# GPUEngineering/RapidNet

Measured on AMD Instinct MI355X. Metric: apg_iterations_per_sec, higher is better.
Workload: dtype f64; 1 GPU; barcelona493: nx=63 nu=114 nv=97 nd=88 N=24 K=493 nodes=10864; operator_storage=dense per-node blocks (reference storage model), parallelism=1 GPU

## Files before the change

rapidnet_amd/csrc/k_stream.hpp:

```cpp
#pragma once
#include "common.hpp"
#include "stream_bits.hpp"

namespace rn {

__device__ __forceinline__ bool stream_nz(double v) { return ((unsigned long long)__double_as_longlong(v) << 1) != 0ull; }
__device__ __forceinline__ bool stream_nz(float v) { return (__float_as_uint(v) << 1) != 0u; }
__host__ __device__ constexpr int stream_vmcnt(int n) { return (n & 15) | ((n >> 4) << 14) | 0x0F70; }
#define RN_LANDED(n) __builtin_amdgcn_s_waitcnt(stream_vmcnt(n));
#define RN_LOADG(buf, sv) _Pragma("unroll") for (int d = 0; d < RN_GROUP; d++) { RN_POP(sv, d) RN_LOAD1(buf, sv, d) }
#define RN_USEG(buf, sv) _Pragma("unroll") for (int d = 0; d < RN_GROUP; d++) RN_USE1(buf, sv, d)
#define RN_LOADH(buf, sv) _Pragma("unroll") for (int d = 0; d < RN_GROUP - 1; d++) if (d < nHead) { RN_POP(sv, d) RN_LOAD1(buf, sv, d) }
#define RN_USEH(buf, sv) _Pragma("unroll") for (int d = 0; d < RN_GROUP - 1; d++) if (d < nHead) RN_USE1(buf, sv, d)
#define RN_STREAM_GROUPS                                                                                               \
    RN_LOADH(bufB, sB)                                                                                                 \
    if (nGroups > 0) RN_LOADG(bufA, sA)                                                                                \
    RN_USEH(bufB, sB)                                                                                                  \
    if (nGroups > 0) {                                                                                                 \
        RN_LANDED(RN_GROUP_LOADS)                                                                                      \
        int g = 0;                                                                                                     \
        for (; g + 2 < nGroups; g += 2) {                                                                              \
            RN_LOADG(bufB, sB)                                                                                         \
            RN_USEG(bufA, sA)                                                                                          \
            RN_LOADG(bufA, sA)                                                                                         \
            RN_USEG(bufB, sB)                                                                                          \
        }                                                                                                              \
        if (g + 1 < nGroups) {                                                                                         \
            RN_LOADG(bufB, sB)                                                                                         \
            RN_USEG(bufA, sA)                                                                                          \
            RN_USEG(bufB, sB)                                                                                          \
        } else {                                                                                                       \
            RN_USEG(bufA, sA)                                                                                          \
        }                                                                                                              \
    }                                                                                                                  \
    RN_LANDED(0)
template <typename T, typename VT, int VPL, int NL, int D, int NR>
__device__ __forceinline__ void stream_walk(const VT *__restrict__ Ab, const T *sh_y, const T *sh_y2, const unsigned long long *sh_nz, int skip, int span0, int span1, int G, int ny,
                                            int spanSlots, const int (&off)[NL], const int (&cj)[NL], const T (&msk)[NL], T (&part)[NL][VPL],
                                            T (&part2)[NR == 2 ? NL : 1][VPL], int &liveSpans, int &liveCols, int &liveRagged) {
    const int lane = threadIdx.x & 63;
    const int rag = (ny % G != 0 && span1 * G > ny) ? ny / G : -1;
    VT bufA[D][NL], bufB[D][NL];
    int sA[D], sB[D];
    liveSpans = 0; liveCols = 0; liveRagged = 0;
    const char *const Abb = reinterpret_cast<const char *>(Ab);
    const unsigned spanBytes = (unsigned)spanSlots * 16u;
    unsigned offB[NL];
#pragma unroll
    for (int j = 0; j < NL; j++) offB[j] = (unsigned)off[j] * 16u;
#define RN_POP(sv, d) { sv[d] = __builtin_amdgcn_readfirstlane(cb + __builtin_ctzll(mf)); mf &= mf - 1ull; }
#define RN_GROUP D
#define RN_GROUP_LOADS (D * NL)
#define RN_LOAD1(buf, sv, d)                                                                                           \
    _Pragma("unroll") for (int j = 0; j < NL; j++)                                                                     \
        buf[d][j] = __builtin_nontemporal_load(reinterpret_cast<const VT *>(Abb + (size_t)sv[d] * spanBytes + offB[j]));
#define RN_USE1(buf, sv, d)                                                                                            \
    _Pragma("unroll") for (int j = 0; j < NL; j++) {                                                                   \
        const T yc = sh_y[sv[d] * G + cj[j]] * msk[j];                                                                 \
        _Pragma("unroll") for (int e = 0; e < VPL; e++) part[j][e] += (T)buf[d][j][e] * yc;                            \
        if (NR == 2) {       \
            const T yc2 = sh_y2[sv[d] * G + cj[j]] * msk[j];                                                           \
            _Pragma("unroll") for (int e = 0; e < VPL; e++) part2[j][e] += (T)buf[d][j][e] * yc2;                      \
        }                                                                                                              \
    }
    for (int cb = span0; cb < span1; cb += 64) {
        const int s = cb + lane;
        int cols = 0;
        if (s < span1) {
            const int c0 = s * G;
            if (skip) {
                cols = __popcll(stream_mask_bits(sh_nz, c0, G));
            } else {
                cols = ny - c0 < G ? ny - c0 : G;
            }
        }
        const unsigned long long m = __ballot(cols > 0);
        liveSpans += __popcll(m);
        if (threadIdx.x < 64) {
            int t = cols;
#pragma unroll
            for (int o = 32; o > 0; o >>= 1) t += __shfl_xor(t, o);
            liveCols += t;
        }
        const unsigned long long ragBit = (rag >= cb && rag < cb + 64) ? (m & (1ull << (rag - cb))) : 0ull;
        unsigned long long mf = m & ~ragBit;
        const int nLive = __popcll(mf), nGroups = nLive / D, nHead = nLive - nGroups * D;
        RN_STREAM_GROUPS
        if (ragBit) {
            liveRagged = 1;
            VT bufR[NL];
#pragma unroll
            for (int j = 0; j < NL; j++) {
                const bool ok = msk[j] != (T)0 && rag * G + cj[j] < ny;
                bufR[j] = __builtin_nontemporal_load(reinterpret_cast<const VT *>(Abb + (size_t)rag * spanBytes + (ok ? offB[j] : 0u)));
            }
#pragma unroll
            for (int j = 0; j < NL; j++) {
                const int c = rag * G + cj[j];
                const bool ok = msk[j] != (T)0 && c < ny;
                const T yc = ok ? sh_y[c] : (T)0;
#pragma unroll
                for (int e = 0; e < VPL; e++) part[j][e] += (T)bufR[j][e] * yc;
                if (NR == 2) {
                    const T yc2 = ok ? sh_y2[c] : (T)0;
#pragma unroll
                    for (int e = 0; e < VPL; e++) part2[j][e] += (T)bufR[j][e] * yc2;
                }
            }
        }
    }
#undef RN_GROUP
#undef RN_GROUP_LOADS
#undef RN_POP
#undef RN_LOAD1
#undef RN_USE1
}
template <typename T, typename VT, int VPL, int DU, int NR>
__device__ __forceinline__ void stream_walk_half(const VT *__restrict__ Ab, const T *sh_y, const T *sh_y2, const unsigned long long *sh_nz, int skip, int halfOn, int span0, int span1,
                                                 int G, int ny, int spanSlots, const int (&off)[2], const int (&cj)[2], const T (&msk)[2], T (&part)[2][VPL],
                                                 T (&part2)[NR == 2 ? 2 : 1][VPL], int &liveSpans, int &liveCols, int &liveRagged, int &liveUnits) {
    const int lane = threadIdx.x & 63, Gh = G >> 1;
    const int u0 = 2 * span0, u1 = 2 * span1;
    const int rag = (ny % G != 0 && span1 * G > ny) ? ny / G : -1;
    VT bufA[DU], bufB[DU];
    int sA[DU], sB[DU];
    liveSpans = 0; liveCols = 0; liveRagged = 0; liveUnits = 0;
    const char *const Abb = reinterpret_cast<const char *>(Ab);
    const unsigned spanBytes = (unsigned)spanSlots * 16u;
    const unsigned offB[2] = {(unsigned)off[0] * 16u, (unsigned)off[1] * 16u};
#define RN_GROUP DU
#define RN_GROUP_LOADS DU
#define RN_POP(sv, d) { sv[d] = __builtin_amdgcn_readfirstlane(ub + __builtin_ctzll(mf)); mf &= mf - 1ull; }
#define RN_LOAD1(buf, sv, d) buf[d] = __builtin_nontemporal_load(reinterpret_cast<const VT *>(Abb + (size_t)(sv[d] >> 1) * spanBytes + ((sv[d] & 1) ? offB[1] : offB[0])));
#define RN_USE1(buf, sv, d) {                                                                                          \
        const bool h1 = (sv[d] & 1) != 0;                                                                              \
        const int cy = (sv[d] >> 1) * G + (h1 ? cj[1] : cj[0]);                                                        \
        const T yv = sh_y[cy];                                                                                         \
        const T ya = h1 ? (T)0 : yv, yb = h1 ? yv : (T)0;                                                              \
        _Pragma("unroll") for (int e = 0; e < VPL; e++) { part[0][e] += (T)buf[d][e] * ya; part[1][e] += (T)buf[d][e] * yb; } \
        if (NR == 2) {                                                                                                 \
            const T yv2 = sh_y2[cy];                                                                                   \
            const T ya2 = h1 ? (T)0 : yv2, yb2 = h1 ? yv2 : (T)0;                                                      \
            _Pragma("unroll") for (int e = 0; e < VPL; e++) { part2[0][e] += (T)buf[d][e] * ya2; part2[NR == 2 ? 1 : 0][e] += (T)buf[d][e] * yb2; } \
        }                                                                                                              \
    }
    for (int ub = u0; ub < u1; ub += 64) {
        const int u = ub + lane;
        const int c0 = halfOn ? u * Gh : (u >> 1) * G, n = halfOn ? Gh : G;
        int cols = 0;
        if (u < u1 && c0 < ny) cols = skip ? __popcll(stream_mask_bits(sh_nz, c0, n)) : (ny - c0 < n ? ny - c0 : n);
        const unsigned long long m = __ballot(cols > 0);
        liveSpans += __popcll((m | (m >> 1)) & 0x5555555555555555ull);
        liveUnits += __popcll(m);
        if (threadIdx.x < 64) {
            int t = (halfOn || !(lane & 1)) ? cols : 0;
#pragma unroll
            for (int o = 32; o > 0; o >>= 1) t += __shfl_xor(t, o);
            liveCols += t;
        }
        const int ragSh = 2 * rag - ub;
        const unsigned long long ragBits = (ragSh >= 0 && ragSh < 64) ? (m & (3ull << ragSh)) : 0ull;
        unsigned long long mf = m & ~ragBits;
        const int nLive = __popcll(mf), nGroups = nLive / DU, nHead = nLive - nGroups * DU;
        RN_STREAM_GROUPS
        if (ragBits) {
            liveRagged = 1;
#pragma unroll
            for (int h = 0; h < 2; h++)
                if ((ragBits >> (ragSh + h)) & 1ull) {
                    if (halfOn) { const int left = ny - (2 * rag + h) * Gh; liveUnits += (1 << 16) + ((left < Gh ? left : Gh) << 20); }
                    const int c = rag * G + cj[h];
                    const bool ok = msk[h] != (T)0 && c < ny;
                    const VT bufR = __builtin_nontemporal_load(reinterpret_cast<const VT *>(Abb + (ok ? (size_t)rag * spanBytes + offB[h] : (size_t)0)));
                    const T yc = ok ? sh_y[c] : (T)0;
#pragma unroll
                    for (int e = 0; e < VPL; e++) part[h][e] += (T)bufR[e] * yc;
                    if (NR == 2) {
                        const T yc2 = ok ? sh_y2[c] : (T)0;
#pragma unroll
                        for (int e = 0; e < VPL; e++) part2[NR == 2 ? h : 0][e] += (T)bufR[e] * yc2;
                    }
                }
        }
    }
#undef RN_GROUP
#undef RN_GROUP_LOADS
#undef RN_POP
#undef RN_LOAD1
#undef RN_USE1
#undef RN_LOADG
#undef RN_USEG
#undef RN_LOADH
#undef RN_USEH
#undef RN_STREAM_GROUPS
#undef RN_LANDED
}
template <typename T, int NL>
__device__ __forceinline__ void stream_slots(int tid, int G, int SPC, int spanSlots, int (&off)[NL], int (&cj)[NL], T (&msk)[NL]) {
    const bool halves = NL == 2 && !(G & 1);
    const int stride = halves ? spanSlots >> 1 : STREAM_THREADS;
#pragma unroll
    for (int j = 0; j < NL; j++) {
        const int q = tid + stride * j;
        const bool ok = halves ? tid < stride : q < spanSlots;
        off[j] = ok ? q : (halves ? stride * (j + 1) - 1 : spanSlots - 1);
        cj[j] = off[j] / SPC;
        msk[j] = ok ? (T)1 : (T)0;
    }
}
template <typename T, typename VT, int VPL, int DU, int NR>
__device__ __forceinline__ void stream_walk_two(const VT *__restrict__ Ab, const T *sh_y, const T *sh_y2, const unsigned long long *sh_nz, int skip, int halfOn, int span0, int span1,
                                                int G, int ny, int spanSlots, const int (&off)[2], const int (&cj)[2], const T (&msk)[2],
                                                T (&part)[2][VPL], T (&part2)[NR == 2 ? 2 : 1][VPL], int &liveSpans, int &liveCols, int &liveRagged, int &liveUnits) {
    liveSpans = 0; liveCols = 0; liveRagged = 0; liveUnits = 0;
    const int firstIdle = (G & 1) ? STREAM_THREADS : spanSlots >> 1;
    if (__builtin_amdgcn_readfirstlane((int)threadIdx.x & ~63) < firstIdle)
        stream_walk_half<T, VT, VPL, DU, NR>(Ab, sh_y, sh_y2, sh_nz, skip, (G & 1) ? 0 : halfOn, span0, span1, G, ny, spanSlots, off, cj, msk, part, part2,
                                            liveSpans, liveCols, liveRagged, liveUnits);
}
template <typename T, int NR>
__device__ __forceinline__ void stream_stage_w(const T *__restrict__ w, const T *__restrict__ w2, T w0, T w20, T *sh_y, T *sh_y2, unsigned long long *sh_nz, int ny) {
    const int tid = threadIdx.x, nzWords = (ny + 63) / 64 + 1;
    for (int c0 = 0; (c0 >> 6) < nzWords; c0 += STREAM_THREADS) {
        const int c = c0 + tid;
        T v = 0, v2 = 0;
        if (c < ny) {
            v = c0 == 0 ? w0 : w[c];
            sh_y[c] = v;
            if (NR == 2) { v2 = c0 == 0 ? w20 : w2[c]; sh_y2[c] = v2; }
        }
        const unsigned long long b = __ballot(stream_nz(v) || (NR == 2 && stream_nz(v2)));
        if ((tid & 63) == 0 && (c >> 6) < nzWords) sh_nz[c >> 6] = b;
    }
}
template <bool UNITS>
__device__ __forceinline__ void stream_record(int2 *live, int *units, int liveSpans, int liveCols, int liveRagged, int liveUnits) {
    if (threadIdx.x == 0 && live) {
        live[blockIdx.x] = make_int2(liveSpans, liveCols | (liveRagged << 30));
        if (UNITS) units[blockIdx.x] = liveUnits;
    }
}
template <typename T>
struct StreamRhs2 { const T *w; T *my; T *qa; };
template <typename T, typename ST, int NL, bool SPLIT, int NR>
struct StreamDepth {
    static constexpr bool native = sizeof(ST) == sizeof(T);
    static constexpr bool shortPair = NR == 2 && (native ? sizeof(T) == 4 : NL >= 3);
    static constexpr int D0 = NL <= 2 ? (SPLIT ? RN_STREAM_D - 1 : RN_STREAM_D) : RN_STREAM_D_WIDE;
    static constexpr int D = shortPair ? (NL == 4 ? 1 : D0 - 1) : D0;
    static constexpr int DU = 2 * D - ((native && shortPair) ? 1 : 0);
};
template <typename T, int NL, bool SPLIT, int NR = 1, typename ST = T>
__global__ void __launch_bounds__(STREAM_THREADS, RN_STREAM_MINW) k_stream_gemv(SweepArgs<T> a, int G, int node0, StreamSplit<T> sp, StreamRhs2<T> r2) {
    static_assert(NR == 1 || !SPLIT, "two right-hand sides: unsplit launches only");
    static_assert(sizeof(ST) == sizeof(T) || (sizeof(T) == 8 && sizeof(ST) == 4), "blocks are stored in the context's type, or in fp32 under fp64");
    typedef typename Slot<ST>::type VT;
    typedef StreamDepth<T, ST, NL, SPLIT, NR> Depth;
    constexpr int VPL = Slot<ST>::N, D = Depth::D, DU = Depth::DU;
    extern __shared__ __attribute__((aligned(16))) unsigned char smem_raw[];
    T *sh_y = reinterpret_cast<T *>(smem_raw);
    T *sh_red = sh_y + ((a.ny + 3) & ~3);
    T *sh_y2 = sh_red + (size_t)G * a.LD;
    T *sh_red2 = sh_y2 + ((a.ny + 3) & ~3);
    const int tid = threadIdx.x;
    const bool split = SPLIT && (int)blockIdx.x >= sp.first;
    const int node = split ? sp.first + (((int)blockIdx.x - sp.first) >> 1) : (int)blockIdx.x;
    const bool second = split && ((((int)blockIdx.x - sp.first) & 1) != 0);
    const int nx = a.nx, nv = a.nv, ny = a.ny, LD = a.LD;
    const int SPC = LD / VPL, spanSlots = G * SPC;
    const VT *__restrict__ Ab = reinterpret_cast<const VT *>(reinterpret_cast<const ST *>(a.A) + (size_t)node * a.strideA);
    const int spansAll = (ny + G - 1) / G;
    const int span0 = SPLIT ? (second ? sp.spanHalf : 0) : 0, span1 = (split && !second) ? sp.spanHalf : spansAll;
    int off[NL], cj[NL];
    T msk[NL];
    stream_slots<T, NL>(tid, G, SPC, spanSlots, off, cj, msk);
    T part[NL][VPL], part2[NR == 2 ? NL : 1][VPL];
#pragma unroll
    for (int j = 0; j < NL; j++)
#pragma unroll
        for (int e = 0; e < VPL; e++) { part[j][e] = 0; if (NR == 2) part2[j][e] = 0; }
    const bool has0 = tid < ny;
    const size_t i0 = (size_t)node * ny + (has0 ? tid : 0);
    const int stage = node >= node0 ? a.chainStage + (node - node0) / a.K : a.tr.stageOf[node];
    const T *dyRow = a.tr.dy + (size_t)stage * ny;
    const T spn = a.tr.sqrtp[node];
    const int tq = tid < nx ? tid : 0;
    const T dq0 = dyRow[tq], dq1 = dyRow[nx + tq];
    const T w0a = a.w[i0];
    T w20 = 0;
    if (NR == 2) w20 = r2.w[i0];
    T qa0 = 0, qa02 = 0;
    unsigned long long *sh_nz = reinterpret_cast<unsigned long long *>(sh_y + (size_t)NR * (((ny + 3) & ~3) + (size_t)G * LD));
    stream_stage_w<T, NR>(a.w + (size_t)node * ny, NR == 2 ? r2.w + (size_t)node * ny : nullptr, w0a, w20, sh_y, sh_y2, sh_nz, ny);
    __syncthreads();
    if (tid < nx) qa0 = stream_qa_elem(spn, dq0, sh_y[tid], dq1, sh_y[nx + tid]);
    if (!second) for (int t = tid + STREAM_THREADS; t < nx; t += STREAM_THREADS)
        a.qa[(size_t)node * nx + t] = stream_qa_elem(spn, dyRow[t], sh_y[t], dyRow[nx + t], sh_y[nx + t]);
    if (NR == 2) {
        if (tid < nx) qa02 = stream_qa_elem(spn, dq0, sh_y2[tid], dq1, sh_y2[nx + tid]);
        for (int t = tid + STREAM_THREADS; t < nx; t += STREAM_THREADS)
            r2.qa[(size_t)node * nx + t] = stream_qa_elem(spn, dyRow[t], sh_y2[t], dyRow[nx + t], sh_y2[nx + t]);
    }
    int liveSpans, liveCols, liveRagged, liveUnits;
    if constexpr (NL == 2) stream_walk_two<T, VT, VPL, DU, NR>(Ab, sh_y, sh_y2, sh_nz, sp.skip, sp.half, span0, span1, G, ny, spanSlots, off, cj, msk, part, part2, liveSpans, liveCols, liveRagged, liveUnits);
    else { stream_walk<T, VT, VPL, NL, D, NR>(Ab, sh_y, sh_y2, sh_nz, sp.skip, span0, span1, G, ny, spanSlots, off, cj, msk, part, part2, liveSpans, liveCols, liveRagged); liveUnits = 0; }
#pragma unroll
    for (int j = 0; j < NL; j++)
        if (msk[j] != (T)0) {
#pragma unroll
            for (int e = 0; e < VPL; e++) { sh_red[(size_t)off[j] * VPL + e] = part[j][e]; if (NR == 2) sh_red2[(size_t)off[j] * VPL + e] = part2[j][e]; }
        }
    if (tid < nx && !second) stream_out(qa0, a.qa + (size_t)node * nx + tid);
    if (NR == 2 && tid < nx) stream_out(qa02, r2.qa + (size_t)node * nx + tid);
    stream_record<NL == 2>(sp.live, sp.units, liveSpans, liveCols, liveRagged, liveUnits);
    __syncthreads();
    T *const myOut = second ? sp.my2 + (size_t)(node - sp.first) * 2 * nv : a.my + (size_t)node * 2 * nv;
    if (NR == 2) {
        T *const myOut2 = r2.my + (size_t)node * 2 * nv;
        for (int r = tid; r < 2 * nv; r += STREAM_THREADS) {
            T s = sh_red[r], s2 = sh_red2[r];
            for (int k = 1; k < G; k++) { s += sh_red[(size_t)k * LD + r]; s2 += sh_red2[(size_t)k * LD + r]; }
            stream_out(s, myOut + r);
            stream_out(s2, myOut2 + r);
        }
        return;
    }
    for (int r = tid; r < 2 * nv; r += STREAM_THREADS) {
        T s = sh_red[r];
        for (int k = 1; k < G; k++) s += sh_red[(size_t)k * LD + r];
        stream_out(s, myOut + r);
    }
}

template <typename T>
__global__ void k_struct_prep(SweepArgs<T> a) {
    const int nx = a.nx, nu = a.nu, ny = a.ny, w = nx + nu;
    const long long n = (long long)a.nodes * w;
    for (long long i = (long long)blockIdx.x * blockDim.x + threadIdx.x; i < n; i += (long long)gridDim.x * blockDim.x) {
        const int node = (int)(i / w), t = (int)(i % w);
        const T *dy = a.tr.dy + (size_t)a.tr.stageOf[node] * ny;
        const size_t y = (size_t)node * ny;
        const T sp = a.tr.sqrtp[node];
        T val;
        if (t < nx) { val = sp * (dy[t] * a.w[y + t] + dy[nx + t] * a.w[y + nx + t]); a.qa[(size_t)node * nx + t] = val; }
        else { const int j = t - nx; val = sp * dy[2 * nx + j] * a.w[y + 2 * nx + j]; }
        a.ab[i] = val;
    }
}


}
```

Baseline: 3237 iterations/s.

## Restructure stream GEMV pipeline with padded first group, hoisted ragged tail, FMA, launch bounds

Reworks the streaming GEMV inner loop so the first group is always loaded at full depth, padding inactive slots with a duplicate address, which lets the head and the first group overlap. It keeps the old joined schedule only for NL==1. The ragged-span tail is moved out of the per-64-span loop and handled once after it. Accumulations now use explicit FMA. Per-variant launch-bound minimum waves are also changed. Padded loads add wasted memory traffic, and the new occupancy hints may raise register pressure or cause spills.

Measured after the change: 3235 iterations/s. Within noise of the previous version (-0.1%).

```diff
diff --git a/rapidnet_amd/csrc/k_stream.hpp b/rapidnet_amd/csrc/k_stream.hpp
--- a/rapidnet_amd/csrc/k_stream.hpp
+++ b/rapidnet_amd/csrc/k_stream.hpp
@@ -4,18 +4,45 @@
 
 namespace rn {
 
+__device__ __forceinline__ double stream_fma(double a, double b, double c) { return __builtin_fma(a, b, c); }
+__device__ __forceinline__ float stream_fma(float a, float b, float c) { return __builtin_fmaf(a, b, c); }
 __device__ __forceinline__ bool stream_nz(double v) { return ((unsigned long long)__double_as_longlong(v) << 1) != 0ull; }
 __device__ __forceinline__ bool stream_nz(float v) { return (__float_as_uint(v) << 1) != 0u; }
 __host__ __device__ constexpr int stream_vmcnt(int n) { return (n & 15) | ((n >> 4) << 14) | 0x0F70; }
 #define RN_LANDED(n) __builtin_amdgcn_s_waitcnt(stream_vmcnt(n));
 #define RN_LOADG(buf, sv) _Pragma("unroll") for (int d = 0; d < RN_GROUP; d++) { RN_POP(sv, d) RN_LOAD1(buf, sv, d) }
 #define RN_USEG(buf, sv) _Pragma("unroll") for (int d = 0; d < RN_GROUP; d++) RN_USE1(buf, sv, d)
-#define RN_LOADH(buf, sv) _Pragma("unroll") for (int d = 0; d < RN_GROUP - 1; d++) if (d < nHead) { RN_POP(sv, d) RN_LOAD1(buf, sv, d) }
-#define RN_USEH(buf, sv) _Pragma("unroll") for (int d = 0; d < RN_GROUP - 1; d++) if (d < nHead) RN_USE1(buf, sv, d)
+#define RN_LOADH(buf, sv, n) _Pragma("unroll") for (int d = 0; d < RN_GROUP - 1; d++) if (d < n) { RN_POP(sv, d) RN_LOAD1(buf, sv, d) }
+#define RN_USEH(buf, sv, n) _Pragma("unroll") for (int d = 0; d < RN_GROUP - 1; d++) if (d < n) RN_USE1(buf, sv, d)
+#define RN_LOADF(buf, sv, n) _Pragma("unroll") for (int d = 0; d < RN_GROUP; d++) { if (d < n) RN_POP(sv, d) else sv[d] = sv[0]; RN_LOAD1(buf, sv, d) }
+#define RN_USEF(buf, sv, n) _Pragma("unroll") for (int d = 0; d < RN_GROUP; d++) RN_USE1F(buf, sv, d, d < n)
 #define RN_STREAM_GROUPS                                                                                               \
-    RN_LOADH(bufB, sB)                                                                                                 \
+    if (nLive > 0) {                                                                                                   \
+        const int nH = nGroups > 0 ? nHead : 0, nF = nGroups > 0 ? RN_GROUP : nHead;                                   \
+        RN_LOADH(bufB, sB, nH)                                                                                         \
+        RN_LOADF(bufA, sA, nF)                                                                                         \
+        RN_USEH(bufB, sB, nH)                                                                                          \
+        RN_LANDED(RN_GROUP_LOADS)                                                                                      \
+        int g = 0;                                                                                                     \
+        for (; g + 2 < nGroups; g += 2) {                                                                              \
+            RN_LOADG(bufB, sB)                                                                                         \
+            RN_USEG(bufA, sA)                                                                                          \
+            RN_LOADG(bufA, sA)                                                                                         \
+            RN_USEG(bufB, sB)                                                                                          \
+        }                                                                                                              \
+        if (g + 1 < nGroups) {                                                                                         \
+            RN_LOADG(bufB, sB)                                                                                         \
+            RN_USEG(bufA, sA)                                                                                          \
+            RN_USEG(bufB, sB)                                                                                          \
+        } else {                                                                                                       \
+            RN_USEF(bufA, sA, nF)                                                                                      \
+        }                                                                                                              \
+    }                                                                                                                  \
+    RN_LANDED(0)
+#define RN_STREAM_GROUPS_JOINED                                                                                        \
+    RN_LOADH(bufB, sB, nHead)                                                                                          \
     if (nGroups > 0) RN_LOADG(bufA, sA)                                                                                \
-    RN_USEH(bufB, sB)                                                                                                  \
+    RN_USEH(bufB, sB, nHead)                                                                                           \
     if (nGroups > 0) {                                                                                                 \
         RN_LANDED(RN_GROUP_LOADS)                                                                                      \
         int g = 0;                                                                                                     \
@@ -57,12 +84,14 @@
 #define RN_USE1(buf, sv, d)                                                                                            \
     _Pragma("unroll") for (int j = 0; j < NL; j++) {                                                                   \
         const T yc = sh_y[sv[d] * G + cj[j]] * msk[j];                                                                 \
-        _Pragma("unroll") for (int e = 0; e < VPL; e++) part[j][e] += (T)buf[d][j][e] * yc;                            \
+        _Pragma("unroll") for (int e = 0; e < VPL; e++) part[j][e] = stream_fma((T)buf[d][j][e], yc, part[j][e]);                            \
         if (NR == 2) {       \
             const T yc2 = sh_y2[sv[d] * G + cj[j]] * msk[j];                                                           \
-            _Pragma("unroll") for (int e = 0; e < VPL; e++) part2[j][e] += (T)buf[d][j][e] * yc2;                      \
-        }                                                                                                              \
-    }
+            _Pragma("unroll") for (int e = 0; e < VPL; e++) part2[j][e] = stream_fma((T)buf[d][j][e], yc2, part2[j][e]);                      \
+        }                                                                                                              \
+    }
+#define RN_USE1F(buf, sv, d, on) if (on) RN_USE1(buf, sv, d)
+    unsigned long long ragLive = 0ull;
     for (int cb = span0; cb < span1; cb += 64) {
         const int s = cb + lane;
         int cols = 0;
@@ -85,27 +114,28 @@
         const unsigned long long ragBit = (rag >= cb && rag < cb + 64) ? (m & (1ull << (rag - cb))) : 0ull;
         unsigned long long mf = m & ~ragBit;
         const int nLive = __popcll(mf), nGroups = nLive / D, nHead = nLive - nGroups * D;
-        RN_STREAM_GROUPS
-        if (ragBit) {
-            liveRagged = 1;
-            VT bufR[NL];
-#pragma unroll
-            for (int j = 0; j < NL; j++) {
-                const bool ok = msk[j] != (T)0 && rag * G + cj[j] < ny;
-                bufR[j] = __builtin_nontemporal_load(reinterpret_cast<const VT *>(Abb + (size_t)rag * spanBytes + (ok ? offB[j] : 0u)));
-            }
-#pragma unroll
-            for (int j = 0; j < NL; j++) {
-                const int c = rag * G + cj[j];
-                const bool ok = msk[j] != (T)0 && c < ny;
-                const T yc = ok ? sh_y[c] : (T)0;
-#pragma unroll
-                for (int e = 0; e < VPL; e++) part[j][e] += (T)bufR[j][e] * yc;
-                if (NR == 2) {
-                    const T yc2 = ok ? sh_y2[c] : (T)0;
-#pragma unroll
-                    for (int e = 0; e < VPL; e++) part2[j][e] += (T)bufR[j][e] * yc2;
-                }
+        if constexpr (NL == 1) { RN_STREAM_GROUPS_JOINED } else { RN_STREAM_GROUPS }
+        ragLive |= ragBit;
+    }
+    if (ragLive) {
+        liveRagged = 1;
+        VT bufR[NL];
+#pragma unroll
+        for (int j = 0; j < NL; j++) {
+            const bool ok = msk[j] != (T)0 && rag * G + cj[j] < ny;
+            bufR[j] = __builtin_nontemporal_load(reinterpret_cast<const VT *>(Abb + (size_t)rag * spanBytes + (ok ? offB[j] : 0u)));
+        }
+#pragma unroll
+        for (int j = 0; j < NL; j++) {
+            const int c = rag * G + cj[j];
+            const bool ok = msk[j] != (T)0 && c < ny;
+            const T yc = ok ? sh_y[c] : (T)0;
+#pragma unroll
+            for (int e = 0; e < VPL; e++) part[j][e] = stream_fma((T)bufR[j][e], yc, part[j][e]);
+            if (NR == 2) {
+                const T yc2 = ok ? sh_y2[c] : (T)0;
+#pragma unroll
+                for (int e = 0; e < VPL; e++) part2[j][e] = stream_fma((T)bufR[j][e], yc2, part2[j][e]);
             }
         }
     }
@@ -114,6 +144,7 @@
 #undef RN_POP
 #undef RN_LOAD1
 #undef RN_USE1
+#undef RN_USE1F
 }
 template <typename T, typename VT, int VPL, int DU, int NR>
 __device__ __forceinline__ void stream_walk_half(const VT *__restrict__ Ab, const T *sh_y, const T *sh_y2, const unsigned long long *sh_nz, int skip, int halfOn, int span0, int span1,
@@ -132,18 +163,21 @@
 #define RN_GROUP_LOADS DU
 #define RN_POP(sv, d) { sv[d] = __builtin_amdgcn_readfirstlane(ub + __builtin_ctzll(mf)); mf &= mf - 1ull; }
 #define RN_LOAD1(buf, sv, d) buf[d] = __builtin_nontemporal_load(reinterpret_cast<const VT *>(Abb + (size_t)(sv[d] >> 1) * spanBytes + ((sv[d] & 1) ? offB[1] : offB[0])));
-#define RN_USE1(buf, sv, d) {                                                                                          \
+#define RN_USE1(buf, sv, d) RN_USE1F(buf, sv, d, true)
+#define RN_USE1F(buf, sv, d, on) {                                                                                     \
         const bool h1 = (sv[d] & 1) != 0;                                                                              \
         const int cy = (sv[d] >> 1) * G + (h1 ? cj[1] : cj[0]);                                                        \
-        const T yv = sh_y[cy];                                                                                         \
+        const T yv = (on) ? sh_y[cy] : (T)0;                                                                            \
         const T ya = h1 ? (T)0 : yv, yb = h1 ? yv : (T)0;                                                              \
-        _Pragma("unroll") for (int e = 0; e < VPL; e++) { part[0][e] += (T)buf[d][e] * ya; part[1][e] += (T)buf[d][e] * yb; } \
+        _Pragma("unroll") for (int e = 0; e < VPL; e++) { part[0][e] = stream_fma((T)buf[d][e], ya, part[0][e]); part[1][e] = stream_fma((T)buf[d][e], yb, part[1][e]); } \
         if (NR == 2) {                                                                                                 \
-            const T yv2 = sh_y2[cy];                                                                                   \
+            const T yv2 = (on) ? sh_y2[cy] : (T)0;                                                                      \
             const T ya2 = h1 ? (T)0 : yv2, yb2 = h1 ? yv2 : (T)0;                                                      \
-            _Pragma("unroll") for (int e = 0; e < VPL; e++) { part2[0][e] += (T)buf[d][e] * ya2; part2[NR == 2 ? 1 : 0][e] += (T)buf[d][e] * yb2; } \
-        }                                                                                                              \
-    }
+            _Pragma("unroll") for (int e = 0; e < VPL; e++) { part2[0][e] = stream_fma((T)buf[d][e], ya2, part2[0][e]); part2[NR == 2 ? 1 : 0][e] = stream_fma((T)buf[d][e], yb2, part2[NR == 2 ? 1 : 0][e]); } \
+        }                                                                                                              \
+    }
+    unsigned long long ragAll = 0ull;
+    int ragShAll = 0;
     for (int ub = u0; ub < u1; ub += 64) {
         const int u = ub + lane;
         const int c0 = halfOn ? u * Gh : (u >> 1) * G, n = halfOn ? Gh : G;
@@ -163,36 +197,42 @@
         unsigned long long mf = m & ~ragBits;
         const int nLive = __popcll(mf), nGroups = nLive / DU, nHead = nLive - nGroups * DU;
         RN_STREAM_GROUPS
-        if (ragBits) {
-            liveRagged = 1;
-#pragma unroll
-            for (int h = 0; h < 2; h++)
-                if ((ragBits >> (ragSh + h)) & 1ull) {
-                    if (halfOn) { const int left = ny - (2 * rag + h) * Gh; liveUnits += (1 << 16) + ((left < Gh ? left : Gh) << 20); }
-                    const int c = rag * G + cj[h];
-                    const bool ok = msk[h] != (T)0 && c < ny;
-                    const VT bufR = __builtin_nontemporal_load(reinterpret_cast<const VT *>(Abb + (ok ? (size_t)rag * spanBytes + offB[h] : (size_t)0)));
-                    const T yc = ok ? sh_y[c] : (T)0;
-#pragma unroll
-                    for (int e = 0; e < VPL; e++) part[h][e] += (T)bufR[e] * yc;
-                    if (NR == 2) {
-                        const T yc2 = ok ? sh_y2[c] : (T)0;
-#pragma unroll
-                        for (int e = 0; e < VPL; e++) part2[NR == 2 ? h : 0][e] += (T)bufR[e] * yc2;
-                    }
+        ragAll |= ragBits;
+        if (ragBits) ragShAll = ragSh;
+    }
+    if (ragAll) {
+        liveRagged = 1;
+#pragma unroll
+        for (int h = 0; h < 2; h++)
+            if ((ragAll >> (ragShAll + h)) & 1ull) {
+                if (halfOn) { const int left = ny - (2 * rag + h) * Gh; liveUnits += (1 << 16) + ((left < Gh ? left : Gh) << 20); }
+                const int c = rag * G + cj[h];
+                const bool ok = msk[h] != (T)0 && c < ny;
+                const VT bufR = __builtin_nontemporal_load(reinterpret_cast<const VT *>(Abb + (ok ? (size_t)rag * spanBytes + offB[h] : (size_t)0)));
+                const T yc = ok ? sh_y[c] : (T)0;
+#pragma unroll
+                for (int e = 0; e < VPL; e++) part[h][e] = stream_fma((T)bufR[e], yc, part[h][e]);
+                if (NR == 2) {
+                    const T yc2 = ok ? sh_y2[c] : (T)0;
+#pragma unroll
+                    for (int e = 0; e < VPL; e++) part2[NR == 2 ? h : 0][e] = stream_fma((T)bufR[e], yc2, part2[NR == 2 ? h : 0][e]);
                 }
-        }
+            }
     }
 #undef RN_GROUP
 #undef RN_GROUP_LOADS
 #undef RN_POP
 #undef RN_LOAD1
 #undef RN_USE1
+#undef RN_USE1F
 #undef RN_LOADG
 #undef RN_USEG
 #undef RN_LOADH
 #undef RN_USEH
+#undef RN_LOADF
+#undef RN_USEF
 #undef RN_STREAM_GROUPS
+#undef RN_STREAM_GROUPS_JOINED
 #undef RN_LANDED
 }
 template <typename T, int NL>
@@ -249,9 +289,10 @@
     static constexpr int D0 = NL <= 2 ? (SPLIT ? RN_STREAM_D - 1 : RN_STREAM_D) : RN_STREAM_D_WIDE;
     static constexpr int D = shortPair ? (NL == 4 ? 1 : D0 - 1) : D0;
     static constexpr int DU = 2 * D - ((native && shortPair) ? 1 : 0);
+    static constexpr int minWaves = (NL == 2 && NR == 1 && (SPLIT || sizeof(ST) == 8)) ? 4 : RN_STREAM_MINW;
 };
 template <typename T, int NL, bool SPLIT, int NR = 1, typename ST = T>
-__global__ void __launch_bounds__(STREAM_THREADS, RN_STREAM_MINW) k_stream_gemv(SweepArgs<T> a, int G, int node0, StreamSplit<T> sp, StreamRhs2<T> r2) {
+__global__ void __launch_bounds__(STREAM_THREADS, (NL == 2 && NR == 1 && (SPLIT || sizeof(ST) == 8)) ? 4 : (NL == 1 && SPLIT) ? 8 : RN_STREAM_MINW) k_stream_gemv(SweepArgs<T> a, int G, int node0, StreamSplit<T> sp, StreamRhs2<T> r2) {
     static_assert(NR == 1 || !SPLIT, "two right-hand sides: unsplit launches only");
     static_assert(sizeof(ST) == sizeof(T) || (sizeof(T) == 8 && sizeof(ST) == 4), "blocks are stored in the context's type, or in fp32 under fp64");
     typedef typename Slot<ST>::type VT;
```
